# ymxlzgy/echoscene

Hardware: AMD Instinct MI355X
Metric: denoising steps/sec (layout+SDF) for 32-node scene-graph, 64^3 SDF (3x16^3 latent), full step = one DDPM layout step + one DDIM shape step over all objects; `value` = the FUSED step (both loops as one hipGraph per step, the layout step on a parallel branch: what the K timed steps ran); `full_steps_p (higher is better)
Workload: dtype f16 MFMA operands / f32 accumulate (shape UNet); f32 (layout, GCN)

## Files before the change

### echoscene_amd/csrc/es_vol.hip

```cpp
#include "es_common.h"
#include <string>
#include <algorithm>
#include <cstdlib>
#include <initializer_list>
#include <utility>
#include <type_traits>

namespace {

__device__ __forceinline__ int f_swz(int row) { return (0x1320 >> (((row >> 2) & 3) * 4)) & 3; }

constexpr int GN_VT = 64;

__global__ __launch_bounds__(256) void k_gn_partial(const es_gn_args a, float* part, int vt) {
    __shared__ float ssum4[4][2048], ssq4[4][2048];
    float* ssum = ssum4[0];
    float* ssq = ssq4[0];
    const int o = blockIdx.y, tile = blockIdx.x, C = a.C1 + a.C2;
    const int v0 = tile * vt;
    const int nv = min(vt, a.V - v0);
    const int c4n = C >> 2;
    const int CX = 64;
    const int cx = threadIdx.x & (CX - 1), vy = threadIdx.x >> 6;
    for (int c4 = cx; c4 < c4n; c4 += CX) {
// ... 729 lines not shown
        const int bias = ntap == 27 ? ((Hi + 1) * Wi + 1) * Cin * 2 : 0;
        rA = __builtin_amdgcn_make_buffer_rsrc((void*)((const char*)Ag - bias), (short)0, (int)OOB, 0x00020000);
        {
            const int t = lane < 27 ? lane : 13;
            const int kd = t / 9 - 1, kh = (t / 3) % 3 - 1, kw = t % 3 - 1;
            dtab = ntap == 27 ? ((kd * Hi + kh) * Wi + kw) * Cin * 2 + bias : 0;
            if (UP_) dtab = ntap == 27 ? (updhw ? 0 : kd * Hi * Wi * Cin * 2) + bias : 0;
        }
#pragma unroll
        for (int j = 0; j < NA; ++j) {
            const int ch = down ? 2 * a_h[j] + p01 : a_h[j];
            const int cw = down ? 2 * a_w[j] + p01 : a_w[j];
            const int cd = downd ? 2 * a_d[j] + p01 : a_d[j];
            voff[j] = (unsigned)(((((long)a_o[j] * Dsrc + cd) * Hi + ch) * Wi + cw) * Cin * 2 + a_lc[j] * 16);
            if (UP_) {
                const int sd = updhw ? a_d[j] >> 1 : a_d[j];
                voff[j] = (unsigned)(((((long)a_o[j] * Di + sd) * Hi + (a_h[j] >> 1)) * Wi + (a_w[j] >> 1)) * Cin * 2 + a_lc[j] * 16);
                const int SD = Hi * Wi * Cin * 2, SH = Wi * Cin * 2, SW = Cin * 2;
                upm[j][0] = (updhw && !(a_d[j] & 1)) ? -SD : 0; upp[j][0] = (updhw && (a_d[j] & 1)) ? SD : 0;
                upm[j][1] = !(a_h[j] & 1) ? -SH : 0;            upp[j][1] = (a_h[j] & 1) ? SH : 0;
                upm[j][2] = !(a_w[j] & 1) ? -SW : 0;            upp[j][2] = (a_w[j] & 1) ? SW : 0;
            }
            unsigned m = 0;
            if (ntap == 1) {
                m = a_ok[j] ? 1u : 0u;
            } else {
                m = a_ok[j] ? tap_mask27(cd, Dsrc, ch, UP_ ? g.H : Hi, cw, UP_ ? g.W : Wi) : 0u;
            }
            msk[j] = m;
        }
    };
    set_phase();
    const unsigned voffB = (unsigned)tid * 16u;

    unsigned sA = 0, sbit = 1;
    int ukd = 0, ukh = 0, ukw = 0;
    auto stage_prep = [&]() __attribute__((always_inline)) {
        sA = (unsigned)__builtin_amdgcn_readlane(dtab, st_tap) + (unsigned)st_c * 64u;
        sbit = 1u << st_tap;
        if (UP_) { ukd = st_tap / 9 - 1; ukh = (st_tap / 3) % 3 - 1; ukw = st_tap % 3 - 1; }
    };
    auto stage_piece = [&](int slot, int pj) __attribute__((always_inline)) {
        char* dst = smem + slot * STAGE_BYTES + wave * 1024;
        if (pj < NA) {
            unsigned vs = voff[pj];
            if (UP_) {
                vs += (unsigned)(ukd < 0 ? upm[pj][0] : ukd > 0 ? upp[pj][0] : 0);
                vs += (unsigned)(ukh < 0 ? upm[pj][1] : ukh > 0 ? upp[pj][1] : 0);
                vs += (unsigned)(ukw < 0 ? upm[pj][2] : ukw > 0 ? upp[pj][2] : 0);
            }
            const unsigned vo = (msk[pj] & sbit) ? vs : OOB;
            __builtin_amdgcn_raw_ptr_buffer_load_lds(rA, (lds_ptr)(dst + pj * (NT * 16)), 16, (int)vo, (int)sA, 0, 0);
        } else {
            const int j = pj - NA;
            const unsigned vB = (unsigned)tid * 16u + (unsigned)j * (NT * 16) >= (unsigned)(BN * BK * 2) ? OOB : voffB;
            __builtin_amdgcn_raw_ptr_buffer_load_lds(rB, (lds_ptr)(dst + A_BYTES + j * (NT * 16)), 16, (int)vB,
                                                     (int)(st_boff + (unsigned)j * (NT * 16)), 0, 0);
        }
    };
    auto stage_advance = [&]() __attribute__((always_inline)) {
        st_boff += (unsigned)B_BYTES;
        if (++st_tap == st_ntap) {
            st_tap = 0;
            if (++st_c == st_kch && !st_phase && a.a2) {
                st_phase = 1; st_c = 0; st_ntap = 1; st_kch = a.Cin2 >> 5; st_boff = 0;
                set_phase();
            }
        }
    };
    auto stage_all = [&](int slot) __attribute__((always_inline)) {
        stage_prep();
#pragma unroll
        for (int pj = 0; pj < NLOAD; ++pj) stage_piece(slot, pj);
        stage_advance();
    };

    f4 acc[MI][7];
#pragma unroll
    for (int i = 0; i < MI; ++i)
#pragma unroll
        for (int j = 0; j < 7; ++j) acc[i][j] = f4{0.f, 0.f, 0.f, 0.f};

    const int i16 = lane & 15, q = lane >> 4;
    const int fragA = (wm * WROWS + i16) * 64 + ((q ^ f_swz(i16)) << 4);
    const int fragB = A_BYTES + (wn * 112 + i16) * 64 + ((q ^ f_swz(i16)) << 4);

    stage_all(0);
    if (nloc > 1) stage_all(1);
    int ks = 0;
    auto body = [&](auto slot_c) __attribute__((always_inline)) {
        constexpr int RS = decltype(slot_c)::value;
        constexpr int WS = (RS + 2) % NS;
        if (ks + 1 < nloc) wait_vmcnt<NLOAD>(); else wait_vmcnt<0>();
        __builtin_amdgcn_s_barrier();
        const bool pf = ks + 2 < nloc;
        if (pf) stage_prep();
        h8 af[MI], bfr[7];
        const char* As = smem + RS * STAGE_BYTES;
#pragma unroll
        for (int j = 0; j < 7; ++j) bfr[j] = *(const h8*)(As + fragB + j * 1024);
#pragma unroll
        for (int i = 0; i < MI; ++i) af[i] = *(const h8*)(As + fragA + i * 1024);
        constexpr int PPR = (NLOAD + MI - 1) / MI;
#pragma unroll
        for (int i = 0; i < MI; ++i) {
#pragma unroll
            for (int j = 0; j < 7; ++j)
                acc[i][j] = __builtin_amdgcn_mfma_f32_16x16x32_f16(af[i], bfr[j], acc[i][j], 0, 0, 0);
            __builtin_amdgcn_sched_barrier(0);
            if (pf) {
#pragma unroll
                for (int pp = 0; pp < PPR; ++pp)
                    if (i * PPR + pp < NLOAD) stage_piece(WS, i * PPR + pp);
            }
            __builtin_amdgcn_sched_barrier(0);
        }
        if (pf) stage_advance();
    };
    while (true) {
        body(std::integral_constant<int, 0>{}); if (++ks >= nloc) break;
// ... 96 lines not shown
template <int NL, int MAXA>
__device__ __forceinline__ void wait_ahead(int ahead) {
    if constexpr (MAXA > 0) {
        if (ahead >= MAXA) { wait_vmcnt<MAXA * NL>(); return; }
        wait_ahead<NL, MAXA - 1>(ahead);
    } else {
        wait_vmcnt<0>();
    }
}

template <int BM_, int NC_, int NP_, bool UP_, int EPI_, bool STATS_, int NS_ = 3>
__device__ __forceinline__ void conv_ws_tile(const es_conv_args& a, const ConvGeom& g, int ncdhw, char* smem, const int wave, const int lane,
                                             const long M, const int bx, const int by, const int ks_begin, const int ks_end,
                                             const int S, const int bz, unsigned long long* stamp) {
    constexpr int NS = NS_, UPS_ = 1;
    constexpr int WROWS = BM_ / (NC_ / 2);
    constexpr int MI = WROWS / 16;
    constexpr int A_BYTES = BM_ * BK * 2, B_BYTES = BNP * BK * 2, UNIT_BYTES = A_BYTES + B_BYTES;
    constexpr int STAGE_BYTES = UPS_ * UNIT_BYTES;
    constexpr int APIECES = BM_ / 16, BPIECES = BNP / 16;
    constexpr int NA = APIECES / NP_, NB = BPIECES / NP_, NLOAD = NA + NB;
    static_assert(APIECES % NP_ == 0 && BPIECES % NP_ == 0, "pieces must divide over the producer waves");
    constexpr unsigned OOB = 0x80000000u;
    typedef __attribute__((address_space(3))) void* lds_ptr;
    (void)stamp;
    const long m0 = (long)bx * BM_;
    const int n0 = by * BN;
    const int kch0 = a.Cin >> 5;
    const int nks0 = a.taps * kch0;
    const int nloc = ks_end - ks_begin;
    const int nstage = (nloc + UPS_ - 1) / UPS_;
    if (wave >= NC_) {
        const int pw = wave - NC_;
        int a_lc[NA], a_o[NA], a_d[NA], a_h[NA], a_w[NA];
        bool a_ok[NA];
#pragma unroll
        for (int j = 0; j < NA; ++j) {
            const int p = (pw + NP_ * j) * 64 + lane;
            const int row = p >> 2;
            a_lc[j] = (p & 3) ^ f_swz(row);
            const long m = m0 + row;
            a_ok[j] = m < M;
            const long mm = a_ok[j] ? m : 0;
            a_w[j] = (int)(mm & (g.W - 1));
            a_h[j] = (int)((mm >> g.lw) & (g.H - 1));
            a_d[j] = (int)((mm >> (g.lw + g.lh)) & (g.D - 1));
            a_o[j] = (int)(mm >> (g.lw + g.lh + g.ld));
        }
        int st_phase = ks_begin >= nks0 ? 1 : 0;
        int st_tap = st_phase ? 0 : ks_begin % a.taps;
        int st_c = st_phase ? (ks_begin - nks0) : (ks_begin / a.taps);
        int st_ntap = st_phase ? 1 : a.taps, st_kch = st_phase ? (a.Cin2 >> 5) : kch0;
        unsigned st_boff = (unsigned)(st_phase ? (ks_begin - nks0) : ks_begin) * (unsigned)B_BYTES;
        unsigned voff[NA], msk[NA];
        int upm[NA][3], upp[NA][3];
        int dtab = 0;
        __amdgpu_buffer_rsrc_t rA, rB;
        auto set_phase = [&]() __attribute__((always_inline)) {
            const _Float16* Wg = (const _Float16*)(st_phase ? a.w2 : a.w);
            const long nks_ph = st_phase ? (long)(a.Cin2 >> 5) : (long)nks0;
            rB = __builtin_amdgcn_make_buffer_rsrc((void*)(Wg + ((long)by * nks_ph) * (BNP * BK)), (short)0, (int)OOB, 0x00020000);
            const _Float16* Ag = (const _Float16*)(st_phase ? a.a2 : a.a);
            const int Cin = st_phase ? a.Cin2 : a.Cin;
            const int p01 = (!st_phase && a.mode == ES_CONV_DOWN_DHW_P01) ? 1 : 0;
            const bool down = !st_phase && (a.mode == ES_CONV_DOWN_HW || a.mode == ES_CONV_DOWN_DHW || p01);
            const bool downd = !st_phase && (a.mode == ES_CONV_DOWN_DHW || p01);
            const int Dsrc = downd ? 2 * g.D : g.D;
            const int Hi = st_phase ? g.H : g.Hi, Wi = st_phase ? g.W : g.Wi;
            const int ntap = st_phase ? 1 : a.taps;
            const bool updhw = UP_ && a.mode == ES_CONV_UP_DHW;
            const int Di = updhw ? g.D / 2 : g.D;
            const int bias = ntap == 27 ? ((Hi + 1) * Wi + 1) * Cin * 2 : 0;
            rA = __builtin_amdgcn_make_buffer_rsrc((void*)((const char*)Ag - bias), (short)0, (int)OOB, 0x00020000);
            {
                const int t = lane < 27 ? lane : 13;
                const int kd = t / 9 - 1, kh = (t / 3) % 3 - 1, kw = t % 3 - 1;
                dtab = ntap == 27 ? ((kd * Hi + kh) * Wi + kw) * Cin * 2 + bias : 0;
                if (UP_) dtab = ntap == 27 ? (updhw ? 0 : kd * Hi * Wi * Cin * 2) + bias : 0;
            }
#pragma unroll
            for (int j = 0; j < NA; ++j) {
                const int ch = down ? 2 * a_h[j] + p01 : a_h[j];
                const int cw = down ? 2 * a_w[j] + p01 : a_w[j];
                const int cd = downd ? 2 * a_d[j] + p01 : a_d[j];
                voff[j] = (unsigned)(((((long)a_o[j] * Dsrc + cd) * Hi + ch) * Wi + cw) * Cin * 2 + a_lc[j] * 16);
                if (UP_) {
                    const int sd = updhw ? a_d[j] >> 1 : a_d[j];
                    voff[j] = (unsigned)(((((long)a_o[j] * Di + sd) * Hi + (a_h[j] >> 1)) * Wi + (a_w[j] >> 1)) * Cin * 2 + a_lc[j] * 16);
                    const int SD = Hi * Wi * Cin * 2, SH = Wi * Cin * 2, SW = Cin * 2;
                    upm[j][0] = (updhw && !(a_d[j] & 1)) ? -SD : 0; upp[j][0] = (updhw && (a_d[j] & 1)) ? SD : 0;
                    upm[j][1] = !(a_h[j] & 1) ? -SH : 0;            upp[j][1] = (a_h[j] & 1) ? SH : 0;
                    upm[j][2] = !(a_w[j] & 1) ? -SW : 0;            upp[j][2] = (a_w[j] & 1) ? SW : 0;
                }
                unsigned m = 0;
                if (ntap == 1) {
                    m = a_ok[j] ? 1u : 0u;
                } else {
                    m = a_ok[j] ? tap_mask27(cd, Dsrc, ch, UP_ ? g.H : Hi, cw, UP_ ? g.W : Wi) : 0u;
                }
                msk[j] = m;
            }
        };
        set_phase();
        ES_STAMP_AT(1);
        const unsigned voffB = (unsigned)lane * 16u;
        auto issue_unit = [&](char* dst) __attribute__((always_inline)) {
            const unsigned sA = (unsigned)__builtin_amdgcn_readlane(dtab, st_tap) + (unsigned)st_c * 64u;
            const unsigned sbit = 1u << st_tap;
            int ukd = 0, ukh = 0, ukw = 0;
            if (UP_) { ukd = st_tap / 9 - 1; ukh = (st_tap / 3) % 3 - 1; ukw = st_tap % 3 - 1; }
#pragma unroll
            for (int j = 0; j < NA; ++j) {
                unsigned vs = voff[j];
                if (UP_) {
                    vs += (unsigned)(ukd < 0 ? upm[j][0] : ukd > 0 ? upp[j][0] : 0);
                    vs += (unsigned)(ukh < 0 ? upm[j][1] : ukh > 0 ? upp[j][1] : 0);
                    vs += (unsigned)(ukw < 0 ? upm[j][2] : ukw > 0 ? upp[j][2] : 0);
                }
                const unsigned vo = (msk[j] & sbit) ? vs : OOB;
                __builtin_amdgcn_raw_ptr_buffer_load_lds(rA, (lds_ptr)(dst + (pw + NP_ * j) * 1024), 16, (int)vo, (int)sA, 0, 0);
            }
#pragma unroll
            for (int j = 0; j < NB; ++j) {
                const int q = pw + NP_ * j;
                const unsigned vB = q * 16 >= BN ? OOB : voffB;
                __builtin_amdgcn_raw_ptr_buffer_load_lds(rB, (lds_ptr)(dst + A_BYTES + q * 1024), 16, (int)vB,
                                                         (int)(st_boff + (unsigned)q * 1024u), 0, 0);
            }
            st_boff += (unsigned)B_BYTES;
            if (++st_tap == st_ntap) {
                st_tap = 0;
                if (++st_c == st_kch && !st_phase && a.a2) {
                    st_phase = 1; st_c = 0; st_ntap = 1; st_kch = a.Cin2 >> 5; st_boff = 0;
                    set_phase();
                }
            }
        };
        int issued = 0;
        auto issue_stage = [&](int st) __attribute__((always_inline)) {
            char* base = smem + (st % NS) * STAGE_BYTES;
#pragma unroll
            for (int u = 0; u < UPS_; ++u)
                if (issued < nloc) { issue_unit(base + u * UNIT_BYTES); ++issued; }
        };
        {
            static_assert(NLOAD * (NS - 2) <= 63, "vmcnt is a 6-bit counter");
#pragma unroll
            for (int st = 0; st < NS - 1; ++st)
                if (st < nstage) issue_stage(st);
            for (int st = 0; st < nstage; ++st) {
                wait_ahead<NLOAD, NS - 2>(nstage - 1 - st);
                __builtin_amdgcn_s_barrier();
                if (st == 0) ES_STAMP_AT(2);
                if (st + NS - 1 < nstage) issue_stage(st + NS - 1);
            }
        }
        ES_STAMP_AT(3);
        f4 dummy[MI][7];
        conv_epilogue<BM_, NC_, false, true, EPI_, false, STATS_>(a, g, dummy, smem, M, m0, n0, wave, lane, S, bz, ncdhw);
        ES_STAMP_AT(4);
        return;
    }
    const int wm = wave >> 1, wn = wave & 1;
    f4 acc[MI][7];
#pragma unroll
    for (int i = 0; i < MI; ++i)
#pragma unroll
        for (int j = 0; j < 7; ++j) acc[i][j] = f4{0.f, 0.f, 0.f, 0.f};
    const int i16 = lane & 15, q = lane >> 4;
    const int fragA = (wm * WROWS + i16) * 64 + ((q ^ f_swz(i16)) << 4);
    const int fragB = A_BYTES + (wn * 112 + i16) * 64 + ((q ^ f_swz(i16)) << 4);
    h8 af[MI], bfr[7];
    {
        int slot = 0;
        ES_STAMP_AT(1);
        __builtin_amdgcn_s_barrier();
        ES_STAMP_AT(2);
        ws_read_frags<MI>(smem, fragA, fragB, af, bfr);
        for (int ks = 0; ks + 1 < nloc; ++ks) {
            slot = slot == NS - 1 ? 0 : slot + 1;
            const char* const An = smem + slot * STAGE_BYTES;
// ... 54 lines not shown
template <int DIR>
__device__ __forceinline__ h8 a3_shift(const h8 v, const bool zero_lane) {
    i4v x = __builtin_bit_cast(i4v, v);
#pragma unroll
    for (int e = 0; e < 4; ++e) {
        const int s = DIR < 0 ? __builtin_amdgcn_update_dpp(0, x[e], 0x111, 0xf, 0xf, true) : __builtin_amdgcn_update_dpp(0, x[e], 0x101, 0xf, 0xf, true);
        x[e] = zero_lane ? 0 : s;
    }
    return __builtin_bit_cast(h8, x);
}

template <bool STATS_>
__global__ __launch_bounds__(768, 3) void k_conv_ws3(const es_conv_args a, const ConvGeom g) {
    constexpr int BM_ = 256, NC_ = 8, NP_ = 4, NSB = 7, MI = 4;
    constexpr int A_BYTES = BM_ * BK * 2, B_BYTES = BNP * BK * 2, A_RING = NSB * B_BYTES;
    constexpr int NA = (BM_ / 16) / NP_, NB = (BNP / 16) / NP_;
    constexpr unsigned OOB = 0x80000000u;
    typedef __attribute__((address_space(3))) void* lds_ptr;
    extern __shared__ __attribute__((aligned(16))) char smem[];
    const int tid = threadIdx.x, lane = tid & 63;
    const int wave = __builtin_amdgcn_readfirstlane(tid >> 6);
    const long M = (long)g.O * g.D * g.H * g.W;
    int bx, by, bz;
    conv_tile_of(a, bx, by, bz);
    const int S = gridDim.z;
    const int kch0 = a.Cin >> 5, nks0 = 27 * kch0;
    int ks_begin, ks_end;
    split_range(nks0, 0, 27, bz, S, ks_begin, ks_end);
    const int nloc = ks_end - ks_begin, ngrp = nloc / 3;
    const long m0 = (long)bx * BM_;
    const int n0 = by * BN;
    if (wave >= NC_) {
        const int pw = wave - NC_;
        unsigned voff[NA], msk[NA];
#pragma unroll
        for (int j = 0; j < NA; ++j) {
            const int p = (pw + NP_ * j) * 64 + lane;
            const int row = p >> 2;
            const int lc = (p & 3) ^ f_swz(row);
            const long m = m0 + row;
            const bool ok = m < M;
            const long mm = ok ? m : 0;
            const int w = (int)(mm & (g.W - 1)), h = (int)((mm >> g.lw) & (g.H - 1)), d = (int)((mm >> (g.lw + g.lh)) & (g.D - 1));
            const int o = (int)(mm >> (g.lw + g.lh + g.ld));
            voff[j] = (unsigned)(((((long)o * g.D + d) * g.H + h) * g.W + w) * a.Cin * 2 + lc * 16);
            msk[j] = ok ? tap_mask27(d, g.D, h, g.H, w, g.W) : 0u;
        }
        const int bias = ((g.H + 1) * g.W + 1) * a.Cin * 2;
        const __amdgpu_buffer_rsrc_t rA = __builtin_amdgcn_make_buffer_rsrc((void*)((const char*)a.a - bias), (short)0, (int)OOB, 0x00020000);
        const __amdgpu_buffer_rsrc_t rB = __builtin_amdgcn_make_buffer_rsrc((void*)((const _Float16*)a.w + ((long)by * nks0) * (BNP * BK)), (short)0, (int)OOB, 0x00020000);
        int dtab;
        {
            const int t = lane < 27 ? lane : 13;
            const int kd = t / 9 - 1, kh = (t / 3) % 3 - 1, kw = t % 3 - 1;
            dtab = ((kd * g.H + kh) * g.W + kw) * a.Cin * 2 + bias;
        }
        int a_tap = ks_begin % 27, a_c = ks_begin / 27;
        unsigned b_off = (unsigned)ks_begin * (unsigned)B_BYTES;
        const unsigned voffB = (unsigned)lane * 16u;
        auto issue_A = [&](int slot) __attribute__((always_inline)) {
            char* dst = smem + A_RING + slot * A_BYTES;
            const unsigned sA = (unsigned)__builtin_amdgcn_readlane(dtab, a_tap + 1) + (unsigned)a_c * 64u;
            const unsigned sbit = 1u << (a_tap + 1);
#pragma unroll
            for (int j = 0; j < NA; ++j)
                __builtin_amdgcn_raw_ptr_buffer_load_lds(rA, (lds_ptr)(dst + (pw + NP_ * j) * 1024), 16, (int)((msk[j] & sbit) ? voff[j] : OOB), (int)sA, 0, 0);
            a_tap += 3;
            if (a_tap == 27) { a_tap = 0; ++a_c; }
        };
        auto issue_B = [&](int slot) __attribute__((always_inline)) {
            char* dst = smem + slot * B_BYTES;
#pragma unroll
            for (int j = 0; j < NB; ++j) {
                const int q = pw + NP_ * j;
                __builtin_amdgcn_raw_ptr_buffer_load_lds(rB, (lds_ptr)(dst + q * 1024), 16, (int)(q * 16 >= BN ? OOB : voffB), (int)(b_off + (unsigned)q * 1024u), 0, 0);
            }
            b_off += (unsigned)B_BYTES;
        };
        int sb = 0;
        auto issue_group = [&](int gi) __attribute__((always_inline)) {
            issue_A(gi & 1);
#pragma unroll
            for (int t = 0; t < 3; ++t) { issue_B(sb); sb = sb == NSB - 1 ? 0 : sb + 1; }
        };
        issue_group(0);
        for (int gi = 0; gi < ngrp; ++gi) {
            wait_vmcnt<0>();
            __builtin_amdgcn_s_barrier();
            if (gi + 1 < ngrp) issue_group(gi + 1);
        }
        __builtin_amdgcn_s_barrier();
        f4 dummy[MI][7];
        conv_epilogue<BM_, NC_, false, true, ES_EPI_NONE, false, STATS_>(a, g, dummy, smem, M, m0, n0, wave, lane, S, bz, 0);
        return;
    }
    const int wm = wave >> 1, wn = wave & 1;
    f4 acc[MI][7];
#pragma unroll
    for (int i = 0; i < MI; ++i)
#pragma unroll
        for (int j = 0; j < 7; ++j) acc[i][j] = f4{0.f, 0.f, 0.f, 0.f};
    const int i16 = lane & 15, q = lane >> 4;
    const int fragA = A_RING + (wm * 64 + i16) * 64 + ((q ^ f_swz(i16)) << 4);
    const int fragB = (wn * 112 + i16) * 64 + ((q ^ f_swz(i16)) << 4);
    const bool zl = (i16 & (g.W - 1)) == 0, zr = (i16 & (g.W - 1)) == ((g.W - 1) & 15);
    h8 afc[MI], bq[3];
    __builtin_amdgcn_s_barrier();
    bq[0] = *(const h8*)(smem + fragB);
    bq[1] = *(const h8*)(smem + fragB + 1024);
#pragma unroll
    for (int i = 0; i < MI; ++i) afc[i] = *(const h8*)(smem + fragA + i * 1024);
    int slotB = 0;
    for (int grp = 0; grp < ngrp; ++grp) {
        const char* const An = smem + ((grp + 1) & 1) * A_BYTES;
        auto unit = [&](auto kwc) __attribute__((always_inline)) {
            constexpr int KW = decltype(kwc)::value;
            const char* const Bc = smem + slotB * B_BYTES;
            slotB = slotB == NSB - 1 ? 0 : slotB + 1;
// ... 45 lines not shown
    const int wave = __builtin_amdgcn_readfirstlane(tid >> 6);
    const long M = (long)g.O * g.D * g.H * g.W;
    int bx, byh, bz;
    {
        const int gx = gridDim.x, gy = gridDim.y;
        const int nwg = gx * gy * (int)gridDim.z;
        const int orig = blockIdx.x + gx * (blockIdx.y + gy * blockIdx.z);
        const int xcd = orig & 7, q = nwg >> 3, r = nwg & 7;
        const int L = (xcd < r ? xcd * (q + 1) : r * (q + 1) + (xcd - r) * q) + (orig >> 3);
        const int per_z = gx * gy;
        bz = L / per_z;
        const int t = L - bz * per_z;
        bx = t % gx;
        byh = t / gx;
    }
    const int by = NCH_ == 2 ? byh : (byh >> 1), half0 = NCH_ == 2 ? 0 : (byh & 1);
    const int S = gridDim.z;
    const long m0 = (long)bx * BM_;
    const int kch0 = a.Cin >> 5;
    const int nks0 = a.taps * kch0;
    int nstage = 0;
#pragma unroll
    for (int s = 0; s < KS_; ++s) {
        int b0, e0;
        split_range(nks0, a.a2 ? (a.Cin2 >> 5) : 0, a.taps, bz * KS_ + s, S * KS_, b0, e0);
        nstage = (e0 - b0) > nstage ? (e0 - b0) : nstage;
    }
    if (wave >= NC_) {
        const int pw = wave - NC_, strm = pw / NPW, sub = pw - strm * NPW;
        int ks_begin, ks_end;
        split_range(nks0, a.a2 ? (a.Cin2 >> 5) : 0, a.taps, bz * KS_ + strm, S * KS_, ks_begin, ks_end);
        const int nloc = ks_end - ks_begin;
        const int npc = (NPIECE - sub + NPW - 1) / NPW;
        int a_lc[JA], a_o[JA], a_d[JA], a_h[JA], a_w[JA];
        bool a_ok[JA];
#pragma unroll
        for (int j = 0; j < JA; ++j) {
            const int p = (sub + NPW * j) * 64 + lane;
            const int row = p >> 2;
            a_lc[j] = (p & 3) ^ f_swz(row);
            const long m = m0 + row;
            a_ok[j] = m < M;
            const long mm = a_ok[j] ? m : 0;
            a_w[j] = (int)(mm & (g.W - 1));
            a_h[j] = (int)((mm >> g.lw) & (g.H - 1));
            a_d[j] = (int)((mm >> (g.lw + g.lh)) & (g.D - 1));
            a_o[j] = (int)(mm >> (g.lw + g.lh + g.ld));
        }
        int st_phase = ks_begin >= nks0 ? 1 : 0;
        int st_tap = st_phase ? 0 : ks_begin % a.taps;
        int st_c = st_phase ? (ks_begin - nks0) : (ks_begin / a.taps);
        int st_ntap = st_phase ? 1 : a.taps, st_kch = st_phase ? (a.Cin2 >> 5) : kch0;
        unsigned st_boff = (unsigned)(st_phase ? (ks_begin - nks0) : ks_begin) * (unsigned)(BNP * BK * 2);
        unsigned voff[JA], msk[JA];
        int upm[JA][3], upp[JA][3];
        int dtab = 0;
        __amdgpu_buffer_rsrc_t rA, rB;
        auto set_phase = [&]() __attribute__((always_inline)) {
            const _Float16* Wg = (const _Float16*)(st_phase ? a.w2 : a.w);
            const long nks_ph = st_phase ? (long)(a.Cin2 >> 5) : (long)nks0;
            rB = __builtin_amdgcn_make_buffer_rsrc((void*)(Wg + ((long)by * nks_ph) * (BNP * BK)), (short)0, (int)OOB, 0x00020000);
            const _Float16* Ag = (const _Float16*)(st_phase ? a.a2 : a.a);
            const int Cin = st_phase ? a.Cin2 : a.Cin;
            const int p01 = (!st_phase && a.mode == ES_CONV_DOWN_DHW_P01) ? 1 : 0;
            const bool down = !st_phase && (a.mode == ES_CONV_DOWN_HW || a.mode == ES_CONV_DOWN_DHW || p01);
            const bool downd = !st_phase && (a.mode == ES_CONV_DOWN_DHW || p01);
            const int Dsrc = downd ? 2 * g.D : g.D;
            const int Hi = st_phase ? g.H : g.Hi, Wi = st_phase ? g.W : g.Wi;
            const int ntap = st_phase ? 1 : a.taps;
            const bool updhw = UP_ && a.mode == ES_CONV_UP_DHW;
            const int Di = updhw ? g.D / 2 : g.D;
            const int bias = ntap == 27 ? ((Hi + 1) * Wi + 1) * Cin * 2 : 0;
            rA = __builtin_amdgcn_make_buffer_rsrc((void*)((const char*)Ag - bias), (short)0, (int)OOB, 0x00020000);
            {
                const int t = lane < 27 ? lane : 13;
                const int kd = t / 9 - 1, kh = (t / 3) % 3 - 1, kw = t % 3 - 1;
                dtab = ntap == 27 ? ((kd * Hi + kh) * Wi + kw) * Cin * 2 + bias : 0;
                if (UP_) dtab = ntap == 27 ? (updhw ? 0 : kd * Hi * Wi * Cin * 2) + bias : 0;
            }
#pragma unroll
            for (int j = 0; j < JA; ++j) {
                const int ch = down ? 2 * a_h[j] + p01 : a_h[j];
                const int cw = down ? 2 * a_w[j] + p01 : a_w[j];
                const int cd = downd ? 2 * a_d[j] + p01 : a_d[j];
                voff[j] = (unsigned)(((((long)a_o[j] * Dsrc + cd) * Hi + ch) * Wi + cw) * Cin * 2 + a_lc[j] * 16);
                if (UP_) {
                    const int sd = updhw ? a_d[j] >> 1 : a_d[j];
                    voff[j] = (unsigned)(((((long)a_o[j] * Di + sd) * Hi + (a_h[j] >> 1)) * Wi + (a_w[j] >> 1)) * Cin * 2 + a_lc[j] * 16);
                    const int SD = Hi * Wi * Cin * 2, SH = Wi * Cin * 2, SW = Cin * 2;
                    upm[j][0] = (updhw && !(a_d[j] & 1)) ? -SD : 0; upp[j][0] = (updhw && (a_d[j] & 1)) ? SD : 0;
                    upm[j][1] = !(a_h[j] & 1) ? -SH : 0;            upp[j][1] = (a_h[j] & 1) ? SH : 0;
                    upm[j][2] = !(a_w[j] & 1) ? -SW : 0;            upp[j][2] = (a_w[j] & 1) ? SW : 0;
                }
                unsigned m = 0;
                if (ntap == 1) m = a_ok[j] ? 1u : 0u;
                else m = a_ok[j] ? tap_mask27(cd, Dsrc, ch, UP_ ? g.H : Hi, cw, UP_ ? g.W : Wi) : 0u;
                msk[j] = m;
            }
        };
        set_phase();
        const unsigned voffB = (unsigned)lane * 16u;
        auto issue_unit = [&](char* dst) __attribute__((always_inline)) {
            const unsigned sA = (unsigned)__builtin_amdgcn_readlane(dtab, st_tap) + (unsigned)st_c * 64u;
            const unsigned sbit = 1u << st_tap;
            int ukd = 0, ukh = 0, ukw = 0;
            if (UP_) { ukd = st_tap / 9 - 1; ukh = (st_tap / 3) % 3 - 1; ukw = st_tap % 3 - 1; }
#pragma unroll
            for (int j = 0; j < JA; ++j) {
                unsigned vs = voff[j];
                if (UP_) {
                    vs += (unsigned)(ukd < 0 ? upm[j][0] : ukd > 0 ? upp[j][0] : 0);
                    vs += (unsigned)(ukh < 0 ? upm[j][1] : ukh > 0 ? upp[j][1] : 0);
                    vs += (unsigned)(ukw < 0 ? upm[j][2] : ukw > 0 ? upp[j][2] : 0);
                }
                const unsigned vo = (msk[j] & sbit) ? vs : OOB;
                __builtin_amdgcn_raw_ptr_buffer_load_lds(rA, (lds_ptr)(dst + (sub + NPW * j) * 1024), 16, (int)vo, (int)sA, 0, 0);
            }
#pragma unroll
            for (int j = JA; j < JMAX; ++j) {
                const int qb = sub + NPW * j - APIECES;
                if (j < JMAX - 1 || qb < BPIECES)
                    __builtin_amdgcn_raw_ptr_buffer_load_lds(rB, (lds_ptr)(dst + A_BYTES + qb * 1024), 16, (int)voffB,
                                                             (int)(st_boff + (unsigned)(half0 * 7 + qb) * 1024u), 0, 0);
            }
            st_boff += (unsigned)(BNP * BK * 2);
            if (++st_tap == st_ntap) {
                st_tap = 0;
                if (++st_c == st_kch && !st_phase && a.a2) {
                    st_phase = 1; st_c = 0; st_ntap = 1; st_kch = a.Cin2 >> 5; st_boff = 0;
                    set_phase();
                }
            }
        };
        auto wait_own = [&](bool more) __attribute__((always_inline)) {
            if (!more) wait_vmcnt<0>();
            else if (npc == JMAX) wait_vmcnt<JMAX>();
            else wait_vmcnt<JMAX - 1>();
        };
        char* const base = smem + strm * UNIT_BYTES;
        if (nloc > 0) issue_unit(base);
        if (nloc > 1) issue_unit(base + STAGE_BYTES);
        for (int st = 0; st < nstage; ++st) {
            if (st < nloc) wait_own(st + 1 < nloc);
            __builtin_amdgcn_s_barrier();
            if (st + 2 < nloc) issue_unit(base + ((st + 2) % NS) * STAGE_BYTES);
        }
        __builtin_amdgcn_s_barrier();
        __builtin_amdgcn_s_barrier();
        f4 dummy[1][7];
        if constexpr (NCH_ == 1) conv_epilogue<64, 8, false, true, EPI_>(a, g, dummy, smem, M, m0, 0, wave, lane, S, bz, ncdhw);
        else { f4 dummy2[2][7]; conv_epilogue<64, 4, false, true, EPI_>(a, g, dummy2, smem, M, m0, 0, wave, lane, S, bz, ncdhw); }
        return;
    }
    const int strm = wave / NCH_, hh = wave - strm * NCH_;
    int ks_begin, ks_end;
    split_range(nks0, a.a2 ? (a.Cin2 >> 5) : 0, a.taps, bz * KS_ + strm, S * KS_, ks_begin, ks_end);
    const int nloc = ks_end - ks_begin;
    constexpr int MI = 4;
    f4 acc[MI][7];
#pragma unroll
    for (int i = 0; i < MI; ++i)
#pragma unroll
        for (int j = 0; j < 7; ++j) acc[i][j] = f4{0.f, 0.f, 0.f, 0.f};
    const int i16 = lane & 15, q = lane >> 4;
    const int fragA = strm * UNIT_BYTES + i16 * 64 + ((q ^ f_swz(i16)) << 4);
    const int fragB = strm * UNIT_BYTES + A_BYTES + hh * (112 * 64) + i16 * 64 + ((q ^ f_swz(i16)) << 4);
    {
        h8 af[MI], bfr[7];
        int slot = 0, done = 0;
        if (nloc > 0) {
            __builtin_amdgcn_s_barrier();
            done = 1;
            ws_read_frags<MI>(smem, fragA, fragB, af, bfr);
// ... 67 lines not shown
    constexpr int A_BYTES = BM_ * BK * 2, B_BYTES = BNP * BK * 2, STAGE_BYTES = A_BYTES + B_BYTES, RING_BYTES = NS * STAGE_BYTES;
    constexpr int NA = (BM_ / 16) / NP_, NB = (BNP / 16) / NP_, NLOAD = NA + NB;
    constexpr unsigned OOB = 0x80000000u;
    typedef __attribute__((address_space(3))) void* lds_ptr;
    extern __shared__ __attribute__((aligned(16))) char smem[];
    const int tid = threadIdx.x, lane = tid & 63;
    const int wave = __builtin_amdgcn_readfirstlane(tid >> 6);
    const long M = (long)g.O * g.D * g.H * g.W;
#ifdef ES_STAMP
    unsigned long long* stamp = g_stamp_buf ? g_stamp_buf + ((size_t)(blockIdx.x + gridDim.x * blockIdx.y) * (NC_ + NP_) + wave) * 8 : nullptr;
#endif
    ES_STAMP_AT(0);
    int bx, byg;
    {
        const int gx = gridDim.x, gy = gridDim.y, nwg = gx * gy;
        const int orig = blockIdx.x + gx * blockIdx.y;
        const int xcd = orig & 7, q = nwg >> 3, r = nwg & 7;
        const int L = (xcd < r ? xcd * (q + 1) : r * (q + 1) + (xcd - r) * q) + (orig >> 3);
        const long slab = (long)a.Cin * BN * 2 * ncb;
        int npanel = (int)(((long)gy * slab + (3L << 20) - 1) / (3L << 20));
        npanel = npanel < 1 ? 1 : (npanel > gy ? gy : npanel);
        const int Pw = (gy + npanel - 1) / npanel, full = gx * Pw;
        const int p = L / full, rr = L - p * full;
        const int w = (gy - p * Pw) < Pw ? (gy - p * Pw) : Pw;
        bx = rr / w;
        byg = p * Pw + (rr - bx * w);
    }
    const long m0 = (long)bx * BM_;
    const int by0 = byg * ncb;
    const int kch = a.Cin >> 5;
    const int total = kch * ncb;
    if (wave >= NC_) {
        const int pw = wave - NC_;
        unsigned voff[NA];
#pragma unroll
        for (int j = 0; j < NA; ++j) {
            const int p = (pw + NP_ * j) * 64 + lane;
            const int row = p >> 2;
            const long m = m0 + row;
            voff[j] = m < M ? (unsigned)(m * a.Cin * 2 + (((p & 3) ^ f_swz(row)) * 16)) : OOB;
        }
        const __amdgpu_buffer_rsrc_t rA = __builtin_amdgcn_make_buffer_rsrc(uniform_ptr(a.a), (short)0, (int)OOB, 0x00020000);
        const _Float16* Wg = (const _Float16*)a.w;
        int cb = 0, c = 0, islot = 0;
        __amdgpu_buffer_rsrc_t rB = __builtin_amdgcn_make_buffer_rsrc(uniform_ptr(Wg + (long)by0 * kch * (BNP * BK)), (short)0, (int)OOB, 0x00020000);
        const unsigned voffB = (unsigned)lane * 16u;
        auto issue = [&]() __attribute__((always_inline)) {
            char* dst = smem + __builtin_amdgcn_readfirstlane(islot) * STAGE_BYTES;
            const unsigned sA = (unsigned)__builtin_amdgcn_readfirstlane(c) * 64u;
            const unsigned sB = (unsigned)__builtin_amdgcn_readfirstlane(c) * (unsigned)B_BYTES;
#pragma unroll
            for (int j = 0; j < NA; ++j)
                __builtin_amdgcn_raw_ptr_buffer_load_lds(rA, (lds_ptr)(dst + (pw + NP_ * j) * 1024), 16, (int)voff[j], (int)sA, 0, 0);
#pragma unroll
            for (int j = 0; j < NB; ++j) {
                const int q = pw + NP_ * j;
                const unsigned vB = q * 16 >= BN ? OOB : voffB;
                __builtin_amdgcn_raw_ptr_buffer_load_lds(rB, (lds_ptr)(dst + A_BYTES + q * 1024), 16, (int)vB, (int)(sB + (unsigned)q * 1024u), 0, 0);
            }
            islot = islot == NS - 1 ? 0 : islot + 1;
            if (++c == kch) {
                c = 0; ++cb;
                rB = __builtin_amdgcn_make_buffer_rsrc(uniform_ptr(Wg + (long)(by0 + cb) * kch * (BNP * BK)), (short)0, (int)OOB, 0x00020000);
            }
        };
        issue();
        if (total > 1) issue();
        if (NS == 4 && total > 2) issue();
        for (int u = 0; u < total; ++u) {
            const int ahead = total - 1 - u < NS - 2 ? total - 1 - u : NS - 2;
            if (ahead >= 2) wait_vmcnt<2 * NLOAD>(); else if (ahead == 1) wait_vmcnt<NLOAD>(); else wait_vmcnt<0>();
            __builtin_amdgcn_s_barrier();
            if (u + NS - 1 < total) issue();
        }
        return;
    }
    const int wm = wave >> 1, wn = wave & 1;
    const int i16 = lane & 15, q = lane >> 4;
    const int fragA = (wm * WROWS + i16) * 64 + ((q ^ f_swz(i16)) << 4);
    const int fragB = A_BYTES + (wn * 112 + i16) * 64 + ((q ^ f_swz(i16)) << 4);
    int slot = 0;
    for (int cb = 0; cb < ncb; ++cb) {
        f4 acc[MI][7];
#pragma unroll
        for (int i = 0; i < MI; ++i)
#pragma unroll
            for (int j = 0; j < 7; ++j) acc[i][j] = f4{0.f, 0.f, 0.f, 0.f};
        h8 af[MI], bfr[7];
        __builtin_amdgcn_s_barrier();
        ws_read_frags<MI>(smem + slot * STAGE_BYTES, fragA, fragB, af, bfr);
        slot = slot == NS - 1 ? 0 : slot + 1;
        for (int ks = 0; ks + 1 < kch; ++ks) {
            const char* const An = smem + slot * STAGE_BYTES;
            slot = slot == NS - 1 ? 0 : slot + 1;
#pragma unroll
            for (int j = 0; j < 7; ++j) acc[0][j] = __builtin_amdgcn_mfma_f32_16x16x32_f16(af[0], bfr[j], acc[0][j], 0, 0, 0);
            __builtin_amdgcn_sched_barrier(0);
            asm volatile("s_waitcnt lgkmcnt(0)" ::: "memory");
            __builtin_amdgcn_s_barrier();
// ... 1272 lines not shown
```

Before: 56.34.

## Issue weight tile loads before A-address setup and precompute phase-2 descriptors

In several conv producer paths, the first B (weight) tile load is now issued before the per-row A address decoding, so weight fetch latency overlaps with index math. The mid-loop phase switch to the second input (a2/w2) no longer calls set_phase; its resource descriptors and offsets are precomputed right after the first A issue, and the switch becomes a register copy. The 27-tap kernel also prefetches three B stages ahead of A setup and simplifies voff math. The cost is extra live registers for the phase-2 state and a reordered issue sequence that the vmcnt accounting must still match.

```diff
diff --git a/echoscene_amd/csrc/es_vol.hip b/echoscene_amd/csrc/es_vol.hip
--- a/echoscene_amd/csrc/es_vol.hip
+++ b/echoscene_amd/csrc/es_vol.hip
@@ -785,6 +785,19 @@
     };
     set_phase();
     const unsigned voffB = (unsigned)tid * 16u;
+    const bool to_phase2 = !UP_ && a.a2 && ks_begin < nks0 && ks_end > nks0;
+    unsigned voff2[NA];
+    __amdgpu_buffer_rsrc_t rA2, rB2;
+    auto prep_phase2 = [&]() __attribute__((always_inline)) {
+        rB2 = __builtin_amdgcn_make_buffer_rsrc((void*)((const _Float16*)a.w2 + ((long)by * (a.Cin2 >> 5)) * (BNP * BK)), (short)0, (int)OOB, 0x00020000);
+        rA2 = __builtin_amdgcn_make_buffer_rsrc((void*)a.a2, (short)0, (int)OOB, 0x00020000);
+#pragma unroll
+        for (int j = 0; j < NA; ++j) {
+            const int p = tid + NT * j;
+            const long m = m0 + (p >> 2);
+            voff2[j] = m < M ? (unsigned)(m * a.Cin2 * 2 + a_lc[j] * 16) : OOB;
+        }
+    };
 
     unsigned sA = 0, sbit = 1;
     int ukd = 0, ukh = 0, ukw = 0;
@@ -815,9 +828,11 @@
         st_boff += (unsigned)B_BYTES;
         if (++st_tap == st_ntap) {
             st_tap = 0;
-            if (++st_c == st_kch && !st_phase && a.a2) {
+            if (++st_c == st_kch && !st_phase && to_phase2) {
                 st_phase = 1; st_c = 0; st_ntap = 1; st_kch = a.Cin2 >> 5; st_boff = 0;
-                set_phase();
+                rA = rA2; rB = rB2; dtab = 0;
+#pragma unroll
+                for (int j = 0; j < NA; ++j) { voff[j] = voff2[j]; msk[j] = 1u; }
             }
         }
     };
@@ -838,7 +853,11 @@
     const int fragA = (wm * WROWS + i16) * 64 + ((q ^ f_swz(i16)) << 4);
     const int fragB = A_BYTES + (wn * 112 + i16) * 64 + ((q ^ f_swz(i16)) << 4);
 
-    stage_all(0);
+    stage_prep();
+#pragma unroll
+    for (int pj = 0; pj < NLOAD; ++pj) stage_piece(0, pj);
+    if (to_phase2) prep_phase2();
+    stage_advance();
     if (nloc > 1) stage_all(1);
     int ks = 0;
     auto body = [&](auto slot_c) __attribute__((always_inline)) {
@@ -1001,6 +1020,32 @@
     const int nstage = (nloc + UPS_ - 1) / UPS_;
     if (wave >= NC_) {
         const int pw = wave - NC_;
+        int st_phase = ks_begin >= nks0 ? 1 : 0;
+        int st_tap = st_phase ? 0 : ks_begin % a.taps;
+        int st_c = st_phase ? (ks_begin - nks0) : (ks_begin / a.taps);
+        int st_ntap = st_phase ? 1 : a.taps, st_kch = st_phase ? (a.Cin2 >> 5) : kch0;
+        unsigned st_boff = (unsigned)(st_phase ? (ks_begin - nks0) : ks_begin) * (unsigned)B_BYTES;
+        unsigned voff[NA], msk[NA];
+        int upm[NA][3], upp[NA][3];
+        int dtab = 0;
+        __amdgpu_buffer_rsrc_t rA, rB;
+        {
+            const _Float16* Wg = (const _Float16*)(st_phase ? a.w2 : a.w);
+            const long nks_ph = st_phase ? (long)(a.Cin2 >> 5) : (long)nks0;
+            rB = __builtin_amdgcn_make_buffer_rsrc((void*)(Wg + ((long)by * nks_ph) * (BNP * BK)), (short)0, (int)OOB, 0x00020000);
+        }
+        const unsigned voffB = (unsigned)lane * 16u;
+        auto issue_B = [&](char* dst) __attribute__((always_inline)) {
+#pragma unroll
+            for (int j = 0; j < NB; ++j) {
+                const int q = pw + NP_ * j;
+                const unsigned vB = q * 16 >= BN ? OOB : voffB;
+                __builtin_amdgcn_raw_ptr_buffer_load_lds(rB, (lds_ptr)(dst + A_BYTES + q * 1024), 16, (int)vB,
+                                                         (int)(st_boff + (unsigned)q * 1024u), 0, 0);
+            }
+        };
+        if (nloc > 0) issue_B(smem);
+        ES_STAMP_AT(5);
         int a_lc[NA], a_o[NA], a_d[NA], a_h[NA], a_w[NA];
         bool a_ok[NA];
 #pragma unroll
@@ -1016,19 +1061,7 @@
             a_d[j] = (int)((mm >> (g.lw + g.lh)) & (g.D - 1));
             a_o[j] = (int)(mm >> (g.lw + g.lh + g.ld));
         }
-        int st_phase = ks_begin >= nks0 ? 1 : 0;
-        int st_tap = st_phase ? 0 : ks_begin % a.taps;
-        int st_c = st_phase ? (ks_begin - nks0) : (ks_begin / a.taps);
-        int st_ntap = st_phase ? 1 : a.taps, st_kch = st_phase ? (a.Cin2 >> 5) : kch0;
-        unsigned st_boff = (unsigned)(st_phase ? (ks_begin - nks0) : ks_begin) * (unsigned)B_BYTES;
-        unsigned voff[NA], msk[NA];
-        int upm[NA][3], upp[NA][3];
-        int dtab = 0;
-        __amdgpu_buffer_rsrc_t rA, rB;
         auto set_phase = [&]() __attribute__((always_inline)) {
-            const _Float16* Wg = (const _Float16*)(st_phase ? a.w2 : a.w);
-            const long nks_ph = st_phase ? (long)(a.Cin2 >> 5) : (long)nks0;
-            rB = __builtin_amdgcn_make_buffer_rsrc((void*)(Wg + ((long)by * nks_ph) * (BNP * BK)), (short)0, (int)OOB, 0x00020000);
             const _Float16* Ag = (const _Float16*)(st_phase ? a.a2 : a.a);
             const int Cin = st_phase ? a.Cin2 : a.Cin;
             const int p01 = (!st_phase && a.mode == ES_CONV_DOWN_DHW_P01) ? 1 : 0;
@@ -1072,8 +1105,20 @@
         };
         set_phase();
         ES_STAMP_AT(1);
-        const unsigned voffB = (unsigned)lane * 16u;
-        auto issue_unit = [&](char* dst) __attribute__((always_inline)) {
+        const bool to_phase2 = !UP_ && a.a2 && ks_begin < nks0 && ks_end > nks0;
+        unsigned voff2[NA];
+        __amdgpu_buffer_rsrc_t rA2, rB2;
+        auto prep_phase2 = [&]() __attribute__((always_inline)) {
+            rB2 = __builtin_amdgcn_make_buffer_rsrc((void*)((const _Float16*)a.w2 + ((long)by * (a.Cin2 >> 5)) * (BNP * BK)), (short)0, (int)OOB, 0x00020000);
+            rA2 = __builtin_amdgcn_make_buffer_rsrc((void*)a.a2, (short)0, (int)OOB, 0x00020000);
+#pragma unroll
+            for (int j = 0; j < NA; ++j) {
+                const int p = (pw + NP_ * j) * 64 + lane;
+                const long m = m0 + (p >> 2);
+                voff2[j] = m < M ? (unsigned)(m * a.Cin2 * 2 + a_lc[j] * 16) : OOB;
+            }
+        };
+        auto issue_A = [&](char* dst) __attribute__((always_inline)) {
             const unsigned sA = (unsigned)__builtin_amdgcn_readlane(dtab, st_tap) + (unsigned)st_c * 64u;
             const unsigned sbit = 1u << st_tap;
             int ukd = 0, ukh = 0, ukw = 0;
@@ -1089,22 +1134,22 @@
                 const unsigned vo = (msk[j] & sbit) ? vs : OOB;
                 __builtin_amdgcn_raw_ptr_buffer_load_lds(rA, (lds_ptr)(dst + (pw + NP_ * j) * 1024), 16, (int)vo, (int)sA, 0, 0);
             }
-#pragma unroll
-            for (int j = 0; j < NB; ++j) {
-                const int q = pw + NP_ * j;
-                const unsigned vB = q * 16 >= BN ? OOB : voffB;
-                __builtin_amdgcn_raw_ptr_buffer_load_lds(rB, (lds_ptr)(dst + A_BYTES + q * 1024), 16, (int)vB,
-                                                         (int)(st_boff + (unsigned)q * 1024u), 0, 0);
-            }
+        };
+        auto advance = [&]() __attribute__((always_inline)) {
             st_boff += (unsigned)B_BYTES;
             if (++st_tap == st_ntap) {
                 st_tap = 0;
-                if (++st_c == st_kch && !st_phase && a.a2) {
+                if (++st_c == st_kch && !st_phase && to_phase2) {
+                    ES_STAMP_AT(6);
                     st_phase = 1; st_c = 0; st_ntap = 1; st_kch = a.Cin2 >> 5; st_boff = 0;
-                    set_phase();
+                    rA = rA2; rB = rB2; dtab = 0;
+#pragma unroll
+                    for (int j = 0; j < NA; ++j) { voff[j] = voff2[j]; msk[j] = 1u; }
+                    ES_STAMP_AT(7);
                 }
             }
         };
+        auto issue_unit = [&](char* dst) __attribute__((always_inline)) { issue_A(dst); issue_B(dst); advance(); };
         int issued = 0;
         auto issue_stage = [&](int st) __attribute__((always_inline)) {
             char* base = smem + (st % NS) * STAGE_BYTES;
@@ -1114,8 +1159,12 @@
         };
         {
             static_assert(NLOAD * (NS - 2) <= 63, "vmcnt is a 6-bit counter");
-#pragma unroll
-            for (int st = 0; st < NS - 1; ++st)
+            static_assert(UPS_ == 1, "the entry order below issues unit 0 = stage 0 by hand");
+            if (nloc > 0) issue_A(smem);
+            if (to_phase2) prep_phase2();
+            if (nloc > 0) { advance(); ++issued; }
+#pragma unroll
+            for (int st = 1; st < NS - 1; ++st)
                 if (st < nstage) issue_stage(st);
             for (int st = 0; st < nstage; ++st) {
                 wait_ahead<NLOAD, NS - 2>(nstage - 1 - st);
@@ -1236,6 +1285,23 @@
     const int n0 = by * BN;
     if (wave >= NC_) {
         const int pw = wave - NC_;
+        const __amdgpu_buffer_rsrc_t rB = __builtin_amdgcn_make_buffer_rsrc((void*)((const _Float16*)a.w + ((long)by * nks0) * (BNP * BK)), (short)0, (int)OOB, 0x00020000);
+        unsigned b_off = (unsigned)ks_begin * (unsigned)B_BYTES;
+        const unsigned voffB = (unsigned)lane * 16u;
+        auto issue_B = [&](int slot) __attribute__((always_inline)) {
+            char* dst = smem + slot * B_BYTES;
+#pragma unroll
+            for (int j = 0; j < NB; ++j) {
+                const int q = pw + NP_ * j;
+                __builtin_amdgcn_raw_ptr_buffer_load_lds(rB, (lds_ptr)(dst + q * 1024), 16, (int)(q * 16 >= BN ? OOB : voffB), (int)(b_off + (unsigned)q * 1024u), 0, 0);
+            }
+            b_off += (unsigned)B_BYTES;
+        };
+        int sb = 0;
+        if (ngrp > 0) {
+#pragma unroll
+            for (int t = 0; t < 3; ++t) { issue_B(sb); ++sb; }
+        }
         unsigned voff[NA], msk[NA];
 #pragma unroll
         for (int j = 0; j < NA; ++j) {
@@ -1246,13 +1312,11 @@
             const bool ok = m < M;
             const long mm = ok ? m : 0;
             const int w = (int)(mm & (g.W - 1)), h = (int)((mm >> g.lw) & (g.H - 1)), d = (int)((mm >> (g.lw + g.lh)) & (g.D - 1));
-            const int o = (int)(mm >> (g.lw + g.lh + g.ld));
-            voff[j] = (unsigned)(((((long)o * g.D + d) * g.H + h) * g.W + w) * a.Cin * 2 + lc * 16);
+            voff[j] = (unsigned)(mm * a.Cin * 2 + lc * 16);
             msk[j] = ok ? tap_mask27(d, g.D, h, g.H, w, g.W) : 0u;
         }
         const int bias = ((g.H + 1) * g.W + 1) * a.Cin * 2;
         const __amdgpu_buffer_rsrc_t rA = __builtin_amdgcn_make_buffer_rsrc((void*)((const char*)a.a - bias), (short)0, (int)OOB, 0x00020000);
-        const __amdgpu_buffer_rsrc_t rB = __builtin_amdgcn_make_buffer_rsrc((void*)((const _Float16*)a.w + ((long)by * nks0) * (BNP * BK)), (short)0, (int)OOB, 0x00020000);
         int dtab;
         {
             const int t = lane < 27 ? lane : 13;
@@ -1260,8 +1324,6 @@
             dtab = ((kd * g.H + kh) * g.W + kw) * a.Cin * 2 + bias;
         }
         int a_tap = ks_begin % 27, a_c = ks_begin / 27;
-        unsigned b_off = (unsigned)ks_begin * (unsigned)B_BYTES;
-        const unsigned voffB = (unsigned)lane * 16u;
         auto issue_A = [&](int slot) __attribute__((always_inline)) {
             char* dst = smem + A_RING + slot * A_BYTES;
             const unsigned sA = (unsigned)__builtin_amdgcn_readlane(dtab, a_tap + 1) + (unsigned)a_c * 64u;
@@ -1272,22 +1334,12 @@
             a_tap += 3;
             if (a_tap == 27) { a_tap = 0; ++a_c; }
         };
-        auto issue_B = [&](int slot) __attribute__((always_inline)) {
-            char* dst = smem + slot * B_BYTES;
-#pragma unroll
-            for (int j = 0; j < NB; ++j) {
-                const int q = pw + NP_ * j;
-                __builtin_amdgcn_raw_ptr_buffer_load_lds(rB, (lds_ptr)(dst + q * 1024), 16, (int)(q * 16 >= BN ? OOB : voffB), (int)(b_off + (unsigned)q * 1024u), 0, 0);
-            }
-            b_off += (unsigned)B_BYTES;
-        };
-        int sb = 0;
         auto issue_group = [&](int gi) __attribute__((always_inline)) {
             issue_A(gi & 1);
 #pragma unroll
             for (int t = 0; t < 3; ++t) { issue_B(sb); sb = sb == NSB - 1 ? 0 : sb + 1; }
         };
-        issue_group(0);
+        if (ngrp > 0) issue_A(0);
         for (int gi = 0; gi < ngrp; ++gi) {
             wait_vmcnt<0>();
             __builtin_amdgcn_s_barrier();
@@ -1399,6 +1451,32 @@
         split_range(nks0, a.a2 ? (a.Cin2 >> 5) : 0, a.taps, bz * KS_ + strm, S * KS_, ks_begin, ks_end);
         const int nloc = ks_end - ks_begin;
         const int npc = (NPIECE - sub + NPW - 1) / NPW;
+        int st_phase = ks_begin >= nks0 ? 1 : 0;
+        int st_tap = st_phase ? 0 : ks_begin % a.taps;
+        int st_c = st_phase ? (ks_begin - nks0) : (ks_begin / a.taps);
+        int st_ntap = st_phase ? 1 : a.taps, st_kch = st_phase ? (a.Cin2 >> 5) : kch0;
+        unsigned st_boff = (unsigned)(st_phase ? (ks_begin - nks0) : ks_begin) * (unsigned)(BNP * BK * 2);
+        unsigned voff[JA], msk[JA];
+        int upm[JA][3], upp[JA][3];
+        int dtab = 0;
+        __amdgpu_buffer_rsrc_t rA, rB;
+        {
+            const _Float16* Wg = (const _Float16*)(st_phase ? a.w2 : a.w);
+            const long nks_ph = st_phase ? (long)(a.Cin2 >> 5) : (long)nks0;
+            rB = __builtin_amdgcn_make_buffer_rsrc((void*)(Wg + ((long)by * nks_ph) * (BNP * BK)), (short)0, (int)OOB, 0x00020000);
+        }
+        const unsigned voffB = (unsigned)lane * 16u;
+        auto issue_B = [&](char* dst) __attribute__((always_inline)) {
+#pragma unroll
+            for (int j = JA; j < JMAX; ++j) {
+                const int qb = sub + NPW * j - APIECES;
+                if (j < JMAX - 1 || qb < BPIECES)
+                    __builtin_amdgcn_raw_ptr_buffer_load_lds(rB, (lds_ptr)(dst + A_BYTES + qb * 1024), 16, (int)voffB,
+                                                             (int)(st_boff + (unsigned)(half0 * 7 + qb) * 1024u), 0, 0);
+            }
+        };
+        char* const base = smem + strm * UNIT_BYTES;
+        if (nloc > 0) issue_B(base);
         int a_lc[JA], a_o[JA], a_d[JA], a_h[JA], a_w[JA];
         bool a_ok[JA];
 #pragma unroll
@@ -1414,19 +1492,7 @@
             a_d[j] = (int)((mm >> (g.lw + g.lh)) & (g.D - 1));
             a_o[j] = (int)(mm >> (g.lw + g.lh + g.ld));
         }
-        int st_phase = ks_begin >= nks0 ? 1 : 0;
-        int st_tap = st_phase ? 0 : ks_begin % a.taps;
-        int st_c = st_phase ? (ks_begin - nks0) : (ks_begin / a.taps);
-        int st_ntap = st_phase ? 1 : a.taps, st_kch = st_phase ? (a.Cin2 >> 5) : kch0;
-        unsigned st_boff = (unsigned)(st_phase ? (ks_begin - nks0) : ks_begin) * (unsigned)(BNP * BK * 2);
-        unsigned voff[JA], msk[JA];
-        int upm[JA][3], upp[JA][3];
-        int dtab = 0;
-        __amdgpu_buffer_rsrc_t rA, rB;
         auto set_phase = [&]() __attribute__((always_inline)) {
-            const _Float16* Wg = (const _Float16*)(st_phase ? a.w2 : a.w);
-            const long nks_ph = st_phase ? (long)(a.Cin2 >> 5) : (long)nks0;
-            rB = __builtin_amdgcn_make_buffer_rsrc((void*)(Wg + ((long)by * nks_ph) * (BNP * BK)), (short)0, (int)OOB, 0x00020000);
             const _Float16* Ag = (const _Float16*)(st_phase ? a.a2 : a.a);
             const int Cin = st_phase ? a.Cin2 : a.Cin;
             const int p01 = (!st_phase && a.mode == ES_CONV_DOWN_DHW_P01) ? 1 : 0;
@@ -1466,8 +1532,20 @@
             }
         };
         set_phase();
-        const unsigned voffB = (unsigned)lane * 16u;
-        auto issue_unit = [&](char* dst) __attribute__((always_inline)) {
+        const bool to_phase2 = !UP_ && a.a2 && ks_begin < nks0 && ks_end > nks0;
+        unsigned voff2[JA];
+        __amdgpu_buffer_rsrc_t rA2, rB2;
+        auto prep_phase2 = [&]() __attribute__((always_inline)) {
+            rB2 = __builtin_amdgcn_make_buffer_rsrc((void*)((const _Float16*)a.w2 + ((long)by * (a.Cin2 >> 5)) * (BNP * BK)), (short)0, (int)OOB, 0x00020000);
+            rA2 = __builtin_amdgcn_make_buffer_rsrc((void*)a.a2, (short)0, (int)OOB, 0x00020000);
+#pragma unroll
+            for (int j = 0; j < JA; ++j) {
+                const int p = (sub + NPW * j) * 64 + lane;
+                const long m = m0 + (p >> 2);
+                voff2[j] = m < M ? (unsigned)(m * a.Cin2 * 2 + a_lc[j] * 16) : OOB;
+            }
+        };
+        auto issue_A = [&](char* dst) __attribute__((always_inline)) {
             const unsigned sA = (unsigned)__builtin_amdgcn_readlane(dtab, st_tap) + (unsigned)st_c * 64u;
             const unsigned sbit = 1u << st_tap;
             int ukd = 0, ukh = 0, ukw = 0;
@@ -1483,29 +1561,28 @@
                 const unsigned vo = (msk[j] & sbit) ? vs : OOB;
                 __builtin_amdgcn_raw_ptr_buffer_load_lds(rA, (lds_ptr)(dst + (sub + NPW * j) * 1024), 16, (int)vo, (int)sA, 0, 0);
             }
-#pragma unroll
-            for (int j = JA; j < JMAX; ++j) {
-                const int qb = sub + NPW * j - APIECES;
-                if (j < JMAX - 1 || qb < BPIECES)
-                    __builtin_amdgcn_raw_ptr_buffer_load_lds(rB, (lds_ptr)(dst + A_BYTES + qb * 1024), 16, (int)voffB,
-                                                             (int)(st_boff + (unsigned)(half0 * 7 + qb) * 1024u), 0, 0);
-            }
+        };
+        auto advance = [&]() __attribute__((always_inline)) {
             st_boff += (unsigned)(BNP * BK * 2);
             if (++st_tap == st_ntap) {
                 st_tap = 0;
-                if (++st_c == st_kch && !st_phase && a.a2) {
+                if (++st_c == st_kch && !st_phase && to_phase2) {
                     st_phase = 1; st_c = 0; st_ntap = 1; st_kch = a.Cin2 >> 5; st_boff = 0;
-                    set_phase();
+                    rA = rA2; rB = rB2; dtab = 0;
+#pragma unroll
+                    for (int j = 0; j < JA; ++j) { voff[j] = voff2[j]; msk[j] = 1u; }
                 }
             }
         };
+        auto issue_unit = [&](char* dst) __attribute__((always_inline)) { issue_A(dst); issue_B(dst); advance(); };
         auto wait_own = [&](bool more) __attribute__((always_inline)) {
             if (!more) wait_vmcnt<0>();
             else if (npc == JMAX) wait_vmcnt<JMAX>();
             else wait_vmcnt<JMAX - 1>();
         };
-        char* const base = smem + strm * UNIT_BYTES;
-        if (nloc > 0) issue_unit(base);
+        if (nloc > 0) issue_A(base);
+        if (to_phase2) prep_phase2();
+        if (nloc > 0) advance();
         if (nloc > 1) issue_unit(base + STAGE_BYTES);
         for (int st = 0; st < nstage; ++st) {
             if (st < nloc) wait_own(st + 1 < nloc);
@@ -1639,6 +1716,21 @@
     const int total = kch * ncb;
     if (wave >= NC_) {
         const int pw = wave - NC_;
+        const _Float16* Wg = (const _Float16*)a.w;
+        int cb = 0, c = 0, islot = 0;
+        __amdgpu_buffer_rsrc_t rB = __builtin_amdgcn_make_buffer_rsrc(uniform_ptr(Wg + (long)by0 * kch * (BNP * BK)), (short)0, (int)OOB, 0x00020000);
+        const unsigned voffB = (unsigned)lane * 16u;
+        auto issue_B = [&]() __attribute__((always_inline)) {
+            char* dst = smem + __builtin_amdgcn_readfirstlane(islot) * STAGE_BYTES;
+            const unsigned sB = (unsigned)__builtin_amdgcn_readfirstlane(c) * (unsigned)B_BYTES;
+#pragma unroll
+            for (int j = 0; j < NB; ++j) {
+                const int q = pw + NP_ * j;
+                const unsigned vB = q * 16 >= BN ? OOB : voffB;
+                __builtin_amdgcn_raw_ptr_buffer_load_lds(rB, (lds_ptr)(dst + A_BYTES + q * 1024), 16, (int)vB, (int)(sB + (unsigned)q * 1024u), 0, 0);
+            }
+        };
+        issue_B();
         unsigned voff[NA];
 #pragma unroll
         for (int j = 0; j < NA; ++j) {
@@ -1648,30 +1740,23 @@
             voff[j] = m < M ? (unsigned)(m * a.Cin * 2 + (((p & 3) ^ f_swz(row)) * 16)) : OOB;
         }
         const __amdgpu_buffer_rsrc_t rA = __builtin_amdgcn_make_buffer_rsrc(uniform_ptr(a.a), (short)0, (int)OOB, 0x00020000);
-        const _Float16* Wg = (const _Float16*)a.w;
-        int cb = 0, c = 0, islot = 0;
-        __amdgpu_buffer_rsrc_t rB = __builtin_amdgcn_make_buffer_rsrc(uniform_ptr(Wg + (long)by0 * kch * (BNP * BK)), (short)0, (int)OOB, 0x00020000);
-        const unsigned voffB = (unsigned)lane * 16u;
-        auto issue = [&]() __attribute__((always_inline)) {
+        auto issue_A = [&]() __attribute__((always_inline)) {
             char* dst = smem + __builtin_amdgcn_readfirstlane(islot) * STAGE_BYTES;
             const unsigned sA = (unsigned)__builtin_amdgcn_readfirstlane(c) * 64u;
-            const unsigned sB = (unsigned)__builtin_amdgcn_readfirstlane(c) * (unsigned)B_BYTES;
 #pragma unroll
             for (int j = 0; j < NA; ++j)
                 __builtin_amdgcn_raw_ptr_buffer_load_lds(rA, (lds_ptr)(dst + (pw + NP_ * j) * 1024), 16, (int)voff[j], (int)sA, 0, 0);
-#pragma unroll
-            for (int j = 0; j < NB; ++j) {
-                const int q = pw + NP_ * j;
-                const unsigned vB = q * 16 >= BN ? OOB : voffB;
-                __builtin_amdgcn_raw_ptr_buffer_load_lds(rB, (lds_ptr)(dst + A_BYTES + q * 1024), 16, (int)vB, (int)(sB + (unsigned)q * 1024u), 0, 0);
-            }
+        };
+        auto advance = [&]() __attribute__((always_inline)) {
             islot = islot == NS - 1 ? 0 : islot + 1;
             if (++c == kch) {
                 c = 0; ++cb;
                 rB = __builtin_amdgcn_make_buffer_rsrc(uniform_ptr(Wg + (long)(by0 + cb) * kch * (BNP * BK)), (short)0, (int)OOB, 0x00020000);
             }
         };
-        issue();
+        auto issue = [&]() __attribute__((always_inline)) { issue_A(); issue_B(); advance(); };
+        issue_A();
+        advance();
         if (total > 1) issue();
         if (NS == 4 && total > 2) issue();
         for (int u = 0; u < total; ++u) {
```

After: 56.60, median of 6. No clear change (+0.5%).
